# JanWosnitza/FrayTracer

Hardware: AMD Instinct MI355X
Metric: Mrays/s (primary+secondary) at 4096x4096; max per-pixel |delta| vs F# ref (delta is measured against the CPU oracle: F# parity is unpinned, DESIGN.md section 2) (higher is better)
Workload: dtype f32

## Files before the change

### fraytracer_amd/csrc/kernels.hip

```cpp
#include <hip/hip_runtime.h>

#include "../../include/fraytracer_hip.h"
#include "ft_device.h"
#include "ft_kernels.h"
#include "ft_math.h"
#include "ft_libm.h"

#define FT_CONST __attribute__((address_space(4)))
typedef const float FT_CONST* cfp;
template <class T> __device__ __forceinline__ const T FT_CONST* as_const(const T* p) {
    return (const T FT_CONST*)(p);
}

__device__ __forceinline__ f3 ld3(cfp c) { return mk3(c[0], c[1], c[2]); }
__device__ __forceinline__ FtInstr ld_instr(const FtInstr FT_CONST* q) {
    FtInstr r; r.op = q->op; r.dst = q->dst; r.src = q->src; r.type = q->type; r.count = q->count; r.data = q->data;
    r.aux = q->aux; r.flags = q->flags; r.f0 = q->f0; r.f1 = q->f1; r.pad0 = 0; r.pad1 = 0; return r;
}
typedef float v4f __attribute__((ext_vector_type(4)));
typedef uint32_t v4u __attribute__((ext_vector_type(4)));
struct ItemRegs { v4f a; v4u b; };
__device__ __forceinline__ ItemRegs ld_item(const FtItemRec FT_CONST* q) {
    ItemRegs r;
    r.a = *reinterpret_cast<const v4f FT_CONST*>(q);
// ... 214 lines not shown
        for (int j = 0; j < FT_UNROLL; ++j) {
            q[j] = ft_sphere_q(prm[j], p);
            if (CLAMP) q[j] = __builtin_fmaxf(q[j], FT_FAST_Q_MIN);
        }
#pragma unroll
        for (int j = 0; j < FT_UNROLL; ++j) sum = sum + ft_exp_fast<NEAR>(ft_strength_times_diff<PW>(si, FT_LOOP_SQRT(q[j]), prm[j].w));
    }
    for (; i < count; ++i) {
        const float4 prm = *reinterpret_cast<const float4*>(ldsC + 4 * i);
        const float q1 = ft_sphere_q(prm, p);
        sum = sum + ft_exp_fast<NEAR>(ft_strength_times_diff<PW>(si, FT_LOOP_SQRT(CLAMP ? __builtin_fmaxf(q1, FT_FAST_Q_MIN) : q1), prm.w));
    }
#ifndef FT_SQRT_5
    if (NEAR) ft_omod_off(mode, sum);
#endif
    return sum;
}

template <bool FMA, bool FQ, bool NEAR = false>
__device__ __forceinline__ float smooth_run_spheres_libm(const float* __restrict__ ldsC, uint32_t count, float si, f3 p, float sum, const ft_u64* __restrict__ tab) {
    uint32_t i = 0;
    for (; i + 4u <= count; i += 4u) {
        float4 prm[4];
        float e[4];
#pragma unroll
        for (int j = 0; j < 4; ++j) prm[j] = *reinterpret_cast<const float4*>(ldsC + 4 * (i + j));
#pragma unroll
        for (int j = 0; j < 4; ++j) {
            const float t = si * (ft_sq<FQ>(ft_sphere_q(prm[j], p)) - prm[j].w);
            e[j] = NEAR ? ft_glibc_expf_main<FMA>(t, tab) : ft_glibc_expf<FMA>(t, tab);
        }
#pragma unroll
        for (int j = 0; j < 4; ++j) sum = sum + e[j];
    }
    for (; i < count; ++i) {
        const float4 prm = *reinterpret_cast<const float4*>(ldsC + 4 * i);
        const float t = si * (ft_sq<FQ>(ft_sphere_q(prm, p)) - prm.w);
        sum = sum + (NEAR ? ft_glibc_expf_main<FMA>(t, tab) : ft_glibc_expf<FMA>(t, tab));
    }
    return sum;
}

__device__ __forceinline__ bool near_point_ok(f3 p, float nearR2) {
    const float pp = p.x * p.x + p.y * p.y + p.z * p.z;
    return __ballot(!(pp <= nearR2)) == 0ull;
}

__device__ __forceinline__ bool fast_point_ok(f3 p, bool active = true) {
    const float m = __builtin_fmaxf(__builtin_fmaxf(__builtin_fabsf(p.x), __builtin_fabsf(p.y)), __builtin_fabsf(p.z));
    const bool bad = !(m < FT_FAST_P_MAX) || p.x != p.x || p.y != p.y || p.z != p.z;
    return __ballot(active && bad) == 0ull;
}

__device__ __forceinline__ void ft_sphere_regime(const FtSceneDev& S, const f3 p, bool& fastOk, bool& nearOk) {
    fastOk = fast_point_ok(p);
    nearOk = fastOk && near_point_ok(p, S.nearR2);
}

#ifdef FT_UNION_PROFILE
__device__ unsigned long long ft_union_dbg[12];
__device__ __forceinline__ void ft_dbg_add(uint32_t k, uint32_t v) {
    __hip_atomic_fetch_add(reinterpret_cast<uint32_t*>(ft_lds) + FT_LDS_CNT_WORDS + threadIdx.x + k * FT_BLOCK, v, __ATOMIC_RELAXED, __HIP_MEMORY_SCOPE_WORKGROUP);
}
__device__ __forceinline__ bool ft_dbg_leader() { return (threadIdx.x & 63u) == (unsigned)(__ffsll((long long)__ballot(1)) - 1); }
__device__ __forceinline__ uint32_t ft_dbg_now() { unsigned long long t; asm volatile("s_memtime %0\n\ts_waitcnt lgkmcnt(0)" : "=s"(t) :: "memory"); return (uint32_t)t; }
#define FT_UDBG(k, v) ft_dbg_add(k, v)
#define FT_UDBG_WAVE(k) do { if (ft_dbg_leader()) ft_dbg_add(k, 64u); } while (0)
#define FT_UDBG_T0(v) const uint32_t v = ft_dbg_now()
#define FT_UDBG_T1(k, v) do { const uint32_t _t = ft_dbg_now(); if (ft_dbg_leader()) ft_dbg_add(k, _t - (v)); } while (0)
#else
#define FT_UDBG(k, v) do {} while (0)
#define FT_UDBG_WAVE(k) do {} while (0)
#define FT_UDBG_T0(v) do {} while (0)
#define FT_UDBG_T1(k, v) do {} while (0)
#endif

__device__ __forceinline__ uint32_t ft_grid_cell(const FtGrid FT_CONST& g, const f3 p) {
    const f3 cc = (p - mk3(g.aabbMin[0], g.aabbMin[1], g.aabbMin[2])) * mk3(g.cellSizeInv[0], g.cellSizeInv[1], g.cellSizeInv[2]);
    const int ix = ft_clamp_i(0, g.count[0] - 1, ft_floor_i(cc.x));
    const int iy = ft_clamp_i(0, g.count[1] - 1, ft_floor_i(cc.y));
    const int iz = ft_clamp_i(0, g.count[2] - 1, ft_floor_i(cc.z));
    return (uint32_t)((ix * g.count[1] + iy) * g.count[2] + iz);
}

template <bool FQ, bool CALLS, class Call>
__device__ __forceinline__ void ft_candidate(uint32_t typeData, uint32_t mat, cfp consts, const f3 p, const float* __restrict__ sd,
                                             const uint32_t* __restrict__ sl, float& d, uint32_t& l, Call call) {
    const uint32_t type = typeData & 15u, data = typeData >> 4;
    if (type == FT_PR_SLOT) { d = sd[data * FT_BLOCK]; l = sl[data * FT_BLOCK]; }
    else if (CALLS && type == FT_PR_CALL) call(data, d, l);
    else { d = prim_eval_t<FQ>(type, pool_at(consts, data), p); l = mat; }
}

template <bool FQ>
__device__ __forceinline__ void eval_union_prims(const FtSceneDev& S, const FtGrid FT_CONST& g, const f3 p,
                                           const float* __restrict__ sd, const uint32_t* __restrict__ sl,
                                           float& outD, uint32_t& outLeaf, float cap, float capBound) {
    FT_UDBG_T0(tWalk);
    const uint32_t cell = g.cellBase + ft_grid_cell(g, p);
    cfp ctr = as_const(S.cellCenters) + 3u * cell;
    const float distanceToCenter = ft_distance(mk3(ctr[0], ctr[1], ctr[2]), p);
    const uint32_t FT_CONST* cellStart = as_const(S.cellStart);
    const FtItemRec FT_CONST* items = as_const(S.items);
    cfp consts = as_const(S.consts);
    uint32_t i = cellStart[cell];
    const uint32_t end = cellStart[cell + 1];
#ifdef FT_UNION_PROFILE
    {
// ... 234 lines not shown
                if constexpr (COOP) {
                    if (fastOk && S.fastQ) eval_union_coop<true, CALLS, MATH>(S, as_const(S.grids)[in.aux], p, sd, sl, ldsC, fastOk, nearOk, d, l);
                    else eval_union_coop<false, CALLS, MATH>(S, as_const(S.grids)[in.aux], p, sd, sl, ldsC, fastOk, nearOk, d, l);
                } else
                {
                    float cap = -__builtin_inff(), capBound = 0.0f;
                    if (in.flags & FT_FLAG_LAZY) {
                        const float d1 = prim_eval(in.type, consts + in.data, p);
                        cfp bd = consts + in.count;
                        if (d1 >= epsHit) { cap = d1; capBound = ft_distance(ld3(bd), p) + bd[3]; }
                    }
                if constexpr (CALLS) {
                    if (fastOk && S.fastQ) eval_union<true, MATH>(S, as_const(S.grids)[in.aux], p, sd, sl, ldsC, fastOk, nearOk, d, l, cap, capBound);
                    else eval_union<false, MATH>(S, as_const(S.grids)[in.aux], p, sd, sl, ldsC, fastOk, nearOk, d, l, cap, capBound);
                } else {
                    if (fastOk && S.fastQ) eval_union_prims<true>(S, as_const(S.grids)[in.aux], p, sd, sl, d, l, cap, capBound);
                    else eval_union_prims<false>(S, as_const(S.grids)[in.aux], p, sd, sl, d, l, cap, capBound);
                }
                }
                *dst = d; sl[in.dst * FT_BLOCK] = l;
            }
            break;
        }
        default: break;
        }
    }
}

template <bool CALLS, int MATH, bool COOP = false>
__device__ __forceinline__ void ft_eval(const FtSceneDev& S, const f3 p, float* __restrict__ sd, uint32_t* __restrict__ sl,
                                        const float* __restrict__ ldsC, float& outD, uint32_t& outLeaf, float epsHit = __builtin_inff(),
                                        const float* __restrict__ cullRow = nullptr, uint32_t cullN = FT_CULL_NONE) {
    const bool fastOk = (S.nStage != 0 || S.fastQ != 0) && fast_point_ok(p);
    const bool nearOk = MATH == 0 && fastOk && S.nStage != 0 && near_point_ok(p, S.nearR2);
    ft_exec<true, CALLS, MATH, COOP>(S, 0u, S.nInstr, p, sd, sl, ldsC, fastOk, nearOk, epsHit, cullRow, cullN);
    outD = sd[0];
    outLeaf = sl[0];
}

#define FT_CULL_MIN 32u
__device__ __forceinline__ f3 ft_readlane3(f3 v, int l) {
    return mk3(__int_as_float(__builtin_amdgcn_readlane(__float_as_int(v.x), l)), __int_as_float(__builtin_amdgcn_readlane(__float_as_int(v.y), l)),
               __int_as_float(__builtin_amdgcn_readlane(__float_as_int(v.z), l)));
}
template <int CTRL> __device__ __forceinline__ float ft_dpp(float old, float v) {
    return __int_as_float(__builtin_amdgcn_update_dpp(__float_as_int(old), __float_as_int(v), CTRL, 0xf, 0xf, false));
}
__device__ __forceinline__ float ft_readlane_f(float v, int l) { return __int_as_float(__builtin_amdgcn_readlane(__float_as_int(v), l)); }
__device__ __forceinline__ float ft_wave_max_all(float v) {
    v = __builtin_fmaxf(v, ft_dpp<0x111>(0.0f, v)); v = __builtin_fmaxf(v, ft_dpp<0x112>(0.0f, v));
    v = __builtin_fmaxf(v, ft_dpp<0x114>(0.0f, v)); v = __builtin_fmaxf(v, ft_dpp<0x118>(0.0f, v));
    return __builtin_fmaxf(__builtin_fmaxf(ft_readlane_f(v, 15), ft_readlane_f(v, 31)), __builtin_fmaxf(ft_readlane_f(v, 47), ft_readlane_f(v, 63)));
}
__device__ __forceinline__ float ft_wave_scan_incl(float v, float& total) {
    const uint32_t lane = threadIdx.x & 63u;
    v += ft_dpp<0x111>(0.0f, v); v += ft_dpp<0x112>(0.0f, v); v += ft_dpp<0x114>(0.0f, v); v += ft_dpp<0x118>(0.0f, v);
    const float r0 = ft_readlane_f(v, 15), r1 = ft_readlane_f(v, 31), r2 = ft_readlane_f(v, 47), r3 = ft_readlane_f(v, 63);
    const float p2 = r0 + r1, p3 = p2 + r2;
    v += lane >= 48u ? p3 : (lane >= 32u ? p2 : (lane >= 16u ? r0 : 0.0f));
    total = p3 + r3;
    return v;
}
__device__ __forceinline__ float ft_wave_shift_right1(float v) { return ft_dpp<0x138>(0.0f, v); }
template <bool HELD = false>
__device__ __forceinline__ uint32_t ft_cull_children(const FtSceneDev& S, const f3 p, bool active, unsigned long long am,
                                                     const float* __restrict__ ldsC, float* __restrict__ row) {
    if (FT_WORD_AT_USE(HELD, S.cullPc) == FT_CULL_NONE) return FT_CULL_NONE;
    const FtInstr FT_CONST* in = as_const(S.instr) + S.cullPc;
    const uint32_t flags = in->flags, count = in->count;
    const float si = in->f0;
    if (in->op != FT_OP_SMOOTH_RUN || !(flags & FT_FLAG_FAST) || count < FT_CULL_MIN || !(si < 0.0f)) return FT_CULL_NONE;
    if (!fast_point_ok(p, active)) return FT_CULL_NONE;
    const uint32_t lane = threadIdx.x & 63u;
    const f3 q00 = ft_readlane3(p, __ffsll((long long)am) - 1);
    const float fx = p.x - q00.x, fy = p.y - q00.y, fz = p.z - q00.z;
    const float far2 = active ? (fx * fx + fy * fy) + fz * fz : 0.0f;
    const float farMax = ft_wave_max_all(far2);
    const unsigned long long fm = __ballot(active && far2 == farMax);
    const f3 q01 = ft_readlane3(p, __ffsll((long long)(fm != 0ull ? fm : am)) - 1);
    const f3 q0 = mk3(0.5f * (q00.x + q01.x), 0.5f * (q00.y + q01.y), 0.5f * (q00.z + q01.z));
    const float ex = p.x - q0.x, ey = p.y - q0.y, ez = p.z - q0.z;
    const float rho2 = ft_wave_max_all(active ? (ex * ex + ey * ey) + ez * ez : 0.0f);
    const float rho = __builtin_amdgcn_sqrtf(rho2) * 1.001f + 1e-6f;
    const uint32_t n = count < FT_CULL_MAX ? count : FT_CULL_MAX;
    const float4* src = reinterpret_cast<const float4*>(ldsC + in->data);
    float4* dst = reinterpret_cast<float4*>(row);
    float carry = 0.0f;
    uint32_t kept = 0;
    bool apart = true;
    for (uint32_t base = 0; base < n; base += 64u) {
        const uint32_t i = base + lane;
        const bool have = i < n;
        const float4 prm = src[have ? i : n - 1u];
        const float dx = prm.x - q0.x, dy = prm.y - q0.y, dz = prm.z - q0.z;
        const float dq = __builtin_amdgcn_sqrtf((dx * dx + dy * dy) + dz * dz);
        const float dc = dq - prm.w;
        if (__ballot(have && !(dq - rho >= 1e-5f * dq + 1e-6f)) != 0ull) apart = false;
        const float slack = 0.01f + rho;
        const float dlo = dc - slack, dhi = dc + slack;
        const float low = have ? __builtin_amdgcn_exp2f(__builtin_fmaxf(si * dhi * 1.44269504f - 0.02f, -200.0f)) : 0.0f;
        float passTotal;
        const float incl = ft_wave_scan_incl(low, passTotal);
        const float excl = ft_wave_shift_right1(incl);
        const float slow = (carry + excl) * 0.99609375f;
        const uint32_t sbits = __float_as_uint(slow);
        const float x = __builtin_fminf(__builtin_fmaxf(si * dlo * 1.44269504f, -1000.0f), 1000.0f);
        const bool drop = have && x == x && sbits >= 0x00800000u && sbits < 0x7f800000u && x + 0.02f <= (float)((int)(sbits >> 23) - 127 - 24);
        const bool keep = have && !drop;
        const unsigned long long km = __ballot(keep);
        if (keep) dst[kept + (uint32_t)__popcll(km & ((1ull << lane) - 1ull))] = prm;
        kept += (uint32_t)__popcll(km);
        carry += passTotal;
    }
    return kept | (apart ? FT_CULL_NOCLAMP : 0u);
}

template <int MATH>
__device__ __forceinline__ float ft_run_spheres(const FtSceneDev& S, const float* __restrict__ c, uint32_t count, float si, const f3 p, float sum0,
                                                bool fastOk, bool nearOk, bool noClamp = false) {
    if (MATH != 0) {
        const ft_u64* tab = ft_libm_tab(S);
        if (S.mathFma) return nearOk ? smooth_run_spheres_libm<true, true, true>(c, count, si, p, sum0, tab)
                            : fastOk ? smooth_run_spheres_libm<true, true>(c, count, si, p, sum0, tab)
                                     : smooth_run_spheres_libm<true, false>(c, count, si, p, sum0, tab);
        return nearOk ? smooth_run_spheres_libm<false, true, true>(c, count, si, p, sum0, tab)
             : fastOk ? smooth_run_spheres_libm<false, true>(c, count, si, p, sum0, tab)
                      : smooth_run_spheres_libm<false, false>(c, count, si, p, sum0, tab);
    }
    if (__builtin_expect(nearOk, 1)) {
#ifndef FT_SQRT_5
        const int pw = ft_strength_pw(si);
        if (noClamp) {
            if (pw == 2) return smooth_run_spheres_fast<true, 2, false>(c, count, si, p, sum0);
            if (pw == 1) return smooth_run_spheres_fast<true, 1, false>(c, count, si, p, sum0);
            if (pw == 3) return smooth_run_spheres_fast<true, 3, false>(c, count, si, p, sum0);
            return smooth_run_spheres_fast<true, 0, false>(c, count, si, p, sum0);
        }
        if (pw == 2) return smooth_run_spheres_fast<true, 2>(c, count, si, p, sum0);
        if (pw == 1) return smooth_run_spheres_fast<true, 1>(c, count, si, p, sum0);
        if (pw == 3) return smooth_run_spheres_fast<true, 3>(c, count, si, p, sum0);
#endif
        return smooth_run_spheres_fast<true>(c, count, si, p, sum0);
    }
    if (fastOk) return smooth_run_spheres_fast<false>(c, count, si, p, sum0);
    float acc = sum0;
    for (uint32_t i = 0; i < count; ++i) acc = acc + ft_exp(si * (ft_distance(mk3(c[4u * i], c[4u * i + 1u], c[4u * i + 2u]), p) - c[4u * i + 3u]));
    return acc;
}

template <int MATH>
__device__ __forceinline__ void ft_eval_smooth_spheres(const FtSceneDev& S, const f3 p, const float* __restrict__ ldsC,
                                                       float& outD, uint32_t& outLeaf, const float* __restrict__ cullRow = nullptr, uint32_t cullN = FT_CULL_NONE) {
    float acc = 0.0f;
    uint32_t leaf = 0;
    bool fastOk, nearOk;
    ft_sphere_regime(S, p, fastOk, nearOk);
    for (uint32_t pc = 0; pc < S.nInstr; ++pc) {
        const FtInstr FT_CONST* in = as_const(S.instr) + pc;
        const uint32_t op = in->op;
        if (op == FT_OP_SMOOTH_RUN) {
            acc = (in->flags & FT_FLAG_INIT) ? 0.0f : acc;
            const bool culled = pc == S.cullPc && cullN != FT_CULL_NONE && fastOk;
            const float* c = culled ? cullRow : ldsC + in->data;
            uint32_t n = culled ? (cullN & 0xffffu) : in->count;
            uint32_t rest = culled && in->count > FT_CULL_MAX ? in->count - FT_CULL_MAX : 0u;
            bool noClamp = culled && (cullN & FT_CULL_NOCLAMP) != 0u;
#pragma nounroll
            for (;;) {
                acc = ft_run_spheres<MATH>(S, c, n, in->f0, p, acc, fastOk, nearOk, noClamp);
                if (rest == 0u) break;
                c = ldsC + in->data + 4u * FT_CULL_MAX; n = rest; rest = 0u; noClamp = false;
            }
        }
        else if (op == FT_OP_SMOOTH_FIN) acc = -ft_log_m<MATH>(acc, S) * in->f0;
        else leaf = in->aux;
    }
    outD = acc; outLeaf = leaf;
}

#define FT_COOP_SEG 256
template <int MATH>
__device__ __forceinline__ float ft_sphere_term(const float4 prm, const f3 p, const float si, const int regime, const FtSceneDev& S) {
    const float q = ft_sphere_q(prm, p);
    if (MATH != 0) {
        const float t = si * ((regime != 0 ? ft_sq<true>(q) : sqrtf(q)) - prm.w);
        return S.mathFma ? ft_glibc_expf<true>(t, ft_libm_tab(S)) : ft_glibc_expf<false>(t, ft_libm_tab(S));
    }
    if (regime == 2) return ft_exp_fast<true>(si * (ft_sq<true>(q) - prm.w));
    if (regime == 1) return ft_exp_fast<false>(si * (ft_sq<true>(q) - prm.w));
    return ft_exp(si * (sqrtf(q) - prm.w));
}
template <int MATH>
__device__ __forceinline__ void ft_eval_smooth_spheres_packed(const FtSceneDev& S, const f3 q, const bool active, const unsigned long long am, const uint32_t nRays,
                                                              const float* __restrict__ ldsC, float* __restrict__ row, float& outD, uint32_t& outLeaf) {
    const uint32_t lane = threadIdx.x & 63u;
    const uint32_t rank = (uint32_t)__popcll(am & ((1ull << lane) - 1ull));
    const uint32_t lg = nRays <= 1u ? 6u : 6u - (32u - (uint32_t)__builtin_clz(nRays - 1u));
    const uint32_t g = 1u << lg;
    auto wave_sync = [] {
        __builtin_amdgcn_fence(__ATOMIC_RELEASE, "wavefront");
        __builtin_amdgcn_wave_barrier();
        __builtin_amdgcn_fence(__ATOMIC_ACQUIRE, "wavefront");
    };
    if (active) { row[3u * rank] = q.x; row[3u * rank + 1u] = q.y; row[3u * rank + 2u] = q.z; }
    wave_sync();
    const uint32_t G = lane >> lg, k = lane & (g - 1u);
    const bool valid = G < nRays;
    const f3 p = valid ? mk3(row[3u * G], row[3u * G + 1u], row[3u * G + 2u]) : mk3(0.0f, 0.0f, 0.0f);
    wave_sync();
// ... 268 lines not shown
    float t0, t1;
    bool ok = ft_cert_segment(S, test, o, dir, eps, len, steps, t0, t1);
    const float A = si * 1.44269504f;
    const float xt = A * (eps + S.certM);
    ok = ok && xt >= -100.0f;
    if (__ballot(ok) == 0ull) return false;
    const float thr = ft_cert_threshold(xt);
    const f3 p0 = ok ? o + dir * t0 : mk3(0.0f, 0.0f, 0.0f);
    const f3 sv = ok ? dir * (t1 - t0) : mk3(1.0f, 0.0f, 0.0f);
    const float iss = 1.0f / ft_dot(sv, sv);
    float sum = 0.0f;
    uint32_t i = 0;
    auto term = [&](const auto prm) { return __builtin_amdgcn_exp2f((__builtin_amdgcn_sqrtf(ft_seg_dist2(prm, p0, sv, iss)) - prm.w) * A); };
    if (S.certK != 0u) {
        const v4f FT_CONST* cl = reinterpret_cast<const v4f FT_CONST*>(as_const(S.certCl));
        const v4f FT_CONST* kid = cl + 2u * S.certK;
        const float mthr = thr * (0.5f / (float)S.certK);
        float all = 0.0f, rest = 0.0f;
        uint32_t mark = 0u;
        for (uint32_t k = 0; k < S.certK; ++k) {
            const float bnd = term(cl[2u * k]) * (float)__float_as_uint(cl[2u * k + 1u].x);
            all += bnd;
            if (bnd >= mthr) mark |= 1u << k;
            else rest += bnd;
        }
        const bool held = ok && all < thr, open = ok && !held;
        if (__ballot(open) == 0ull) return held;
        float exact = 0.0f;
        for (uint32_t k = 0; k < S.certK; ++k) {
            const bool mine = (mark >> k) & 1u;
            if (__ballot(open && mine) == 0ull) continue;
            const v4f r = cl[2u * k + 1u];
            const uint32_t cnt = __float_as_uint(r.x), first = __float_as_uint(r.y);
            float part = 0.0f;
            for (uint32_t j = 0; j < cnt; ++j) part += term(kid[first + j]);
            exact += mine ? part : 0.0f;
            if (__ballot(open && exact < thr) == 0ull) return held;
        }
        return held || (open && rest + exact < thr);
    }
    for (; i + 8u <= n; i += 8u) {
#pragma unroll
        for (int j = 0; j < 8; ++j) sum += term(c[i + j]);
        if (__ballot(ok && sum < thr) == 0ull) return false;
    }
    for (; i < n; ++i) sum += term(c[i]);
    return ok && sum < thr;
}

__device__ __forceinline__ int ft_axis_lane(unsigned long long mm) {
    return (mm >> 27) != 0ull ? 26 + __ffsll((long long)(mm >> 27)) : __ffsll((long long)mm) - 1;
}

__device__ __forceinline__ bool ft_bundle_certificate(const FtSceneDev& S, const float* __restrict__ ldsC, bool cand, const f3 o, const f3 dir, float eps, float len,
                                                      uint32_t steps, uint32_t minMembers) {
    float t0, t1;
    const bool mem = ft_cert_segment(S, cand, o, dir, eps, len, steps, t0, t1);
    const unsigned long long mm = __ballot(mem);
    if (mm == 0ull || (uint32_t)__popcll(mm) < minMembers) return false;
    const FtInstr FT_CONST* in = as_const(S.instr);
    const float A = in->f0 * 1.44269504f;
    const uint32_t n = in->count;
    const float4* c = reinterpret_cast<const float4*>(ldsC + in->data);
    const int ax = ft_axis_lane(mm);
    const f3 oc = ft_readlane3(o, ax), dc = ft_readlane3(dir, ax);
    const float tc0 = ft_readlane_f(t0, ax), tc1 = ft_readlane_f(t1, ax);
    const f3 g = o - oc, h = dir - dc;
    const float sl = ft_dot(g, dc) * (1.0f / ft_dot(dc, dc));
    const float ex = __builtin_fmaf(-sl, dc.x, g.x), ey = __builtin_fmaf(-sl, dc.y, g.y), ez = __builtin_fmaf(-sl, dc.z, g.z);
    const float al = __builtin_amdgcn_sqrtf(__builtin_fmaf(ez, ez, __builtin_fmaf(ey, ey, ex * ex)));
    const float bl = __builtin_amdgcn_sqrtf(__builtin_fmaf(h.z, h.z, __builtin_fmaf(h.y, h.y, h.x * h.x)));
    const float Wr = ft_wave_max_all(mem ? __builtin_fmaf(bl, t1, al) : 0.0f);
    const float epsMax = ft_wave_max_all(mem ? eps : 0.0f);
    const float Rc = (S.escR + epsMax + S.certClip) * 1.001f;
    const float W = Wr * 1.001f + (1e-6f + 4e-6f * Rc);
    const float xt = A * (epsMax + S.certM);
    if (!(W <= S.escR) || !(xt >= -100.0f)) return false;
    const float dLo = ft_wave_max_all(mem ? __builtin_fmaxf(tc1 - (sl + t0), 0.0f) : 0.0f);
    const float dHi = ft_wave_max_all(mem ? __builtin_fmaxf((sl + t1) - tc0, 0.0f) : 0.0f);
    const float i0 = (tc1 - dLo) - 4e-6f * Rc, i1 = (tc0 + dHi) + 4e-6f * Rc;
    const f3 p0 = oc + dc * i0, sv = dc * (i1 - i0);
    const float iss = 1.0f / ft_dot(sv, sv);
    const float thr = ft_cert_threshold(xt);
    const uint32_t lane = threadIdx.x & 63u;
    float sum = 0.0f;
    for (uint32_t base = 0; base < n; base += 64u) {
        const uint32_t i = base + lane;
        const float4 prm = c[i < n ? i : n - 1u];
        const float term = __builtin_amdgcn_exp2f((__builtin_amdgcn_sqrtf(ft_seg_dist2(prm, p0, sv, iss)) - (prm.w + W)) * A);
        sum += i < n ? term : 0.0f;
    }
    float total;
    ft_wave_scan_incl(sum, total);
    return mem && total < thr;
}

__device__ __forceinline__ bool ft_occlusion_certificate(const FtRenderArgs& a, const float* __restrict__ ldsC, bool cand, const f3 o, const f3 dir, float eps, float len,
                                                         uint32_t steps) {
    const FtSceneDev& S = a.S;
    const f3 w = o - mk3(S.escC[0], S.escC[1], S.escC[2]);
    const float dd = ft_dot(dir, dir);
    const bool ok = cand && a.occ.b >= 0.0f && S.escR >= 0.0f && eps >= a.occ.epsMin && eps <= S.escR && len > 0.0f && len < 1e9f && dd >= 0.81f && dd <= 1.000001f &&
                    ft_dot(w, w) <= S.certRho2 && steps < FT_STEP_CAP / 2u;
    const unsigned long long mm = __ballot(ok);
    if (mm == 0ull) return false;
    const FtInstr FT_CONST* in = as_const(S.instr);
    const uint32_t n = in->count;
    const float si = in->f0;
    const float4* c = reinterpret_cast<const float4*>(ldsC + in->data);
    const float tEnd = len * a.occ.lenInv;
    const int ax = ft_axis_lane(mm);
    const f3 oc = ft_readlane3(o, ax), dc = ft_readlane3(dir, ax);
    const float tc = ft_readlane_f(tEnd, ax), idc = 1.0f / ft_dot(dc, dc);
    const uint32_t lane = threadIdx.x & 63u;
    auto approach = [](const f3 p, const f3 q, const f3 e, const float ie, const float tMaxi, float& t) {
        const float vx = p.x - q.x, vy = p.y - q.y, vz = p.z - q.z;
        t = __builtin_amdgcn_fmed3f(__builtin_fmaf(vz, e.z, __builtin_fmaf(vy, e.y, vx * e.x)) * ie, 0.0f, tMaxi);
        const float ex = __builtin_fmaf(-t, e.x, vx), ey = __builtin_fmaf(-t, e.y, vy), ez = __builtin_fmaf(-t, e.z, vz);
        return __builtin_amdgcn_sqrtf(__builtin_fmaf(ez, ez, __builtin_fmaf(ey, ey, ex * ex)));
    };
    float best = 0.0f, tAx;
    uint32_t bi = 0u;
    for (uint32_t base = 0; base < n; base += 64u) {
        const uint32_t i = base + lane;
        const float4 prm = c[i < n ? i : n - 1u];
        const float nr = (prm.w + a.occ.near) - approach(mk3(prm.x, prm.y, prm.z), oc, dc, idc, tc, tAx);
        if (i < n && nr > best) { best = nr; bi = i; }
    }
    const float nearest = ft_wave_max_all(best);
    if (!(nearest > 0.0f)) return false;
    const int src = __ffsll((long long)__ballot(best == nearest)) - 1;
    const float4 sp = c[(uint32_t)__builtin_amdgcn_readlane((int)bi, src)];
    (void)approach(mk3(sp.x, sp.y, sp.z), oc, dc, idc, tc, tAx);
    const f3 y = oc + dc * tAx;
    const float A = si * 1.44269504f;
    float sum = 0.0f;
    for (uint32_t base = 0; base < n; base += 64u) {
        const uint32_t i = base + lane;
        const float4 prm = c[i < n ? i : n - 1u];
        const float dx = prm.x - y.x, dy = prm.y - y.y, dz = prm.z - y.z;
        const float term = __builtin_amdgcn_exp2f((__builtin_amdgcn_sqrtf(__builtin_fmaf(dz, dz, __builtin_fmaf(dy, dy, dx * dx))) - prm.w) * A);
        sum += i < n ? term : 0.0f;
    }
    float total;
    ft_wave_scan_incl(sum, total);
    const float D = __builtin_amdgcn_logf(total) * (-0.693147181f / si);
    const float ie = 1.0f / eps, idd = 1.0f / dd;
    float t;
    bool holds = false;
    {
        const float dist = approach(mk3(sp.x, sp.y, sp.z), o, dir, idd, tEnd, t);
        const float nSteps = __builtin_fmaf(t, ie, 2.0f), hitM = __builtin_fmaf(a.occ.e, nSteps, a.occ.b);
        holds = t <= a.occ.reach && nSteps < 131072.0f && hitM <= a.occ.cap && (dist + hitM) * 1.001f < sp.w;
    }
    {
        const float dist = approach(y, o, dir, idd, tEnd, t);
        const float nSteps = __builtin_fmaf(t, ie, 2.0f), hitM = __builtin_fmaf(a.occ.e, nSteps, a.occ.b);
        holds = holds || (t <= a.occ.reach && nSteps < 131072.0f && hitM <= a.occ.cap && (dist + hitM) * 1.001f < D);
    }
    return ok && holds;
}

__device__ __forceinline__ int first_step_from_cache(LaneState& s) {
    if (s.len <= 0.0f) return 0;
    const float d = *ft_sh(FT_SH_D0);
    if (d != d) { ft_flag(1u); return 2; }
    if (d < s.eps) return 1;
    s.o = s.o + s.dir * d;
    s.len = s.len - d;
    s.steps = 1;
    return 0;
}

struct FtLit { f3 lint, ldir; };
__device__ __forceinline__ FtLit ft_light_at(const uint32_t type, const f3 lv, const f3 lc, const f3 hp) {
    f3 lint = lc, ldir = lv;
    if (type != FT_LIGHT_DIRECTIONAL) { ldir = ft_normalize(lv - hp); lint = lint / ft_length2(lv - hp); }
    return FtLit{lint, ldir};
}

template <bool EXT, int FORM = FT_FORM_FRAME, bool LEAN = false>
__device__ __forceinline__ void settle(const FtRenderArgs& a, LaneState& s) {
// ... 284 lines not shown
            const unsigned long long idle = __ballot(s.phase == PH_IDLE);
            if (idle == 0ull) break;
            if ((uint32_t)__popcll(idle) < a.refillMin && __ballot(s.phase >= PH_MARCH) != 0ull) break;
            if (chunkNext == chunkEnd) {
                if (exhausted) break;
                const FtRenderArgs& u = FT_ARGS_AT_USE(LEAN, a);
                if (ORDER && u.tileCost != nullptr && lane == 0) {
                    const uint32_t t = tileSt[0];
                    if (t < (u.nJobs >> 6)) u.tileCost[t] = waveEvals - tileSt[TILE_EVALS];
                    tileSt[0] = 0xffffffffu;
                }
                uint32_t base = 0, take = u.chunk;
                if (lane == 0) {
                    if (u.shrink1 < u.nJobs) {
                        const uint32_t cur = __hip_atomic_load(u.counter, __ATOMIC_RELAXED, __HIP_MEMORY_SCOPE_AGENT);
                        take = cur >= u.shrink2 ? u.chunk / 4u : (cur >= u.shrink1 ? u.chunk / 2u : u.chunk);
                    }
                    base = atomicAdd(u.counter, take);
                }
                base = __builtin_amdgcn_readfirstlane(base);
                const uint32_t took = (uint32_t)__builtin_amdgcn_readfirstlane((int)take);
                if (base >= u.nJobs) { exhausted = true; break; }
                chunkNext = base;
                chunkEnd = (u.nJobs - base < took) ? u.nJobs : base + took;
                if (ORDER && u.tileCost != nullptr) {
                    uint32_t tile = base >> 6;
                    if (u.tileOrder != nullptr) {
                        tile = (uint32_t)__builtin_amdgcn_readfirstlane((int)u.tileOrder[tile]);
                        chunkNext = tile << 6; chunkEnd = chunkNext + 64u;
                    }
                    if (lane == 0) { tileSt[0] = tile; tileSt[TILE_EVALS] = waveEvals; }
                }
            }
            uint32_t avail = chunkEnd - chunkNext;
            if (VIEWS && a.mode == 0u) {
                const uint32_t jobsPerView = a.jobsPerPlane * (EXT ? a.spp : 1u);
                const uint32_t v = chunkNext / jobsPerView, viewEnd = (v + 1u) * jobsPerView;
                if (viewEnd - chunkNext < avail) avail = viewEnd - chunkNext;
                cfp c = as_const(a.views) + 12u * v;
                vc.o = ld3(c); vc.fw = ld3(c + 3); vc.up = ld3(c + 6); vc.rt = ld3(c + 9);
                vc.d = ft_readlane_f(dCam, (int)v); vc.leaf = (uint32_t)__builtin_amdgcn_readlane((int)leafCam, (int)v);
            }
            const uint32_t nIdle = (uint32_t)__popcll(idle);
            const uint32_t rank = (uint32_t)__popcll(idle & ((1ull << lane) - 1ull));
            if (s.phase == PH_IDLE && rank < avail) { s.job = chunkNext + rank; start_job<EXT, FORM, LEAN>(a, s, camKnown, dCam, leafCam, vc); }
            chunkNext += (nIdle < avail) ? nIdle : avail;
        }
        if (s.phase == PH_IDLE && exhausted && chunkNext == chunkEnd) s.phase = PH_DONE;
        if (__ballot(s.phase != PH_DONE) == 0ull) break;

        if (VARIANT == 1 && FT_WORD_AT_USE(LEAN, a.occPeriod) != 0u && waveEvals % a.occPeriod == 0u) {
            const bool cand = s.phase == PH_SHADOW && s.steps - a.occFrom < a.occPeriod && (!EXT || !s.inside());
            if ((uint32_t)__popcll(__ballot(cand)) >= a.occMin) {
                const bool hit = ft_occlusion_certificate(FT_ARGS_AT_USE(LEAN, a), ldsC + 0, cand, s.o, s.dir, s.eps, s.len, s.steps);
                if (hit) { ft_count(FT_C_HITS); s.lidx += 1; s.phase = PH_LIGHTS; settle<EXT, FORM, LEAN>(a, s); }
                if (__ballot(hit) != 0ull && __ballot(s.phase >= PH_MARCH) == 0ull) continue;
            }
        }

        if (VARIANT == 1 && FT_WORD_AT_USE(LEAN, a.cert) != 0u) {
            bool ends = false;
            if (FT_WORD_AT_USE(LEAN, a.bundlePeriod) != 0u && waveEvals % a.bundlePeriod == 0u) {
#pragma unroll 1
                for (uint32_t ph = SHADE ? PH_SHADOW : PH_MARCH; ph <= PH_SHADOW; ph += PH_SHADOW - PH_MARCH) {
                    const bool cand = s.phase == ph && (ph == PH_MARCH || s.steps >= a.bundleShadow) && (!EXT || !s.inside());
                    if ((uint32_t)__popcll(__ballot(cand)) < a.bundleMin) continue;
                    if (ft_bundle_certificate(FT_ARGS_AT_USE(LEAN, a).S, ldsC + 0, cand, s.o, s.dir, s.eps, s.len, s.steps, a.bundleMin)) ends = true;
                }
            }
            const bool due = !ends && (s.phase == PH_MARCH || s.phase == PH_SHADOW) && s.steps >= s.certAt && (!EXT || !s.inside());
            bool tried = false;
            if ((uint32_t)__popcll(__ballot(due)) >= a.certMin) {
                tried = true;
                const FtRenderArgs& u = FT_ARGS_AT_USE(LEAN, a);
                const bool holds = ft_miss_certificate(u.S, ldsC + 0, due, s.o, s.dir, s.eps, s.len, s.steps);
                if (due) {
                    if (holds) ends = true;
                    else s.certAt = u.certRepeat != 0u ? s.steps + u.certRepeat : 0xffffffffu;
                }
            }
            if (ends) { s.len = -1.0f; settle<EXT, FORM, LEAN>(a, s); }
            if ((tried || __ballot(ends) != 0ull) && __ballot(s.phase >= PH_MARCH) == 0ull) continue;
        }

        const bool active = s.phase >= PH_MARCH;
        waveEvals += 1;
        FT_UDBG_T0(tRound);
        auto query_point = [&]() {
            f3 q = s.o;
            if (!SHADE && s.phase >= PH_NX && s.phase <= PH_NC) {
                const f3 base = s.o + s.dir * (-s.eps);
                const float h = s.eps * 0.125f;
                q = base;
                if (s.phase == PH_NX) q.x = base.x + h;
                if (s.phase == PH_NY) q.y = base.y + h;
                if (s.phase == PH_NZ) q.z = base.z + h;
            }
            return q;
        };
        const unsigned long long am = __ballot(active);
        const bool camRound = __ballot(s.phase == PH_CAM) != 0ull;
        if (LEAN) { if (!camRound) ft_wave_word_add(waveSt + ST_EVALS, (uint32_t)__popcll(am)); }
        else if (!camRound) nEvals += (uint32_t)__popcll(am);
        const bool coop = (uint32_t)__popcll(am) <= a.tailK;
        float dCoop = 0.0f; uint32_t leafCoop = 0;
        if (coop && am != 0ull) {
            const f3 qm = query_point();
            if (VARIANT == 1) {
                ft_eval_smooth_spheres_packed<MATH>(a.S, qm, active, am, (uint32_t)__popcll(am), ldsC, coopRow, dCoop, leafCoop);
                if (LEAN) { if (!camRound) ft_wave_word_add(waveSt + ST_COOP, (uint32_t)__popcll(am)); }
                else if (!camRound) coopEvals += (uint32_t)__popcll(am);
            } else {
                unsigned long long m = am;
                while (m != 0ull) {
                    const int L = __ffsll((long long)m) - 1;
                    m &= m - 1ull;
                    const f3 qL = ft_readlane3(qm, L);
                    float dL; uint32_t leafL;
                    if (VARIANT == 3) ft_eval_carved<K, true>(a.S, a.carve, qL, dL, leafL, __builtin_inff());
                    else ft_eval<VARIANT == 2, MATH, true>(a.S, qL, sd, sl, ldsC, dL, leafL);
                    if ((int)lane == L) { dCoop = dL; leafCoop = leafL; }
                    if (!camRound) coopEvals += 1;
                }
            }
        }
        uint32_t cullN = FT_CULL_NONE;
        if (VARIANT != 3 && FT_WORD_AT_USE(LEAN, a.cull) != 0u && !coop && am != 0ull) {
            cullN = ft_cull_children<LEAN>(a.S, query_point(), active, am, ldsC, coopRow);
            if (cullN != FT_CULL_NONE) {
                const uint32_t cnt = (as_const(a.S.instr) + a.S.cullPc)->count;
                const uint32_t looked = cnt < FT_CULL_MAX ? cnt : FT_CULL_MAX;
                const uint32_t total = looked * (uint32_t)__popcll(am) >> 6, skipped = (looked - (cullN & 0xffffu)) * (uint32_t)__popcll(am) >> 6;
                if (LEAN) { ft_wave_word_add(waveSt + ST_CULL_TOTAL, total); ft_wave_word_add(waveSt + ST_CULL_SKIPPED, skipped); }
                else { cullTotal += total; cullSkipped += skipped; }
            }
        }
        if (active) {
            float d; uint32_t leaf;
            FT_UDBG_T0(tEval);
            if (coop) { d = dCoop; leaf = leafCoop; }
            else {
                const f3 q = query_point();
                if (VARIANT == 1) ft_eval_smooth_spheres<MATH>(a.S, q, ldsC, d, leaf, coopRow, cullN);
                else if (VARIANT == 3) ft_eval_carved<K>(a.S, a.carve, q, d, leaf, a.lazy == 0u ? __builtin_inff() : s.eps);
                else ft_eval<VARIANT == 2, MATH>(a.S, q, sd, sl, ldsC, d, leaf,
                                                  (EXT && s.inside()) || a.lazy == 0u ? __builtin_inff() : s.eps, coopRow, cullN);
            }
            FT_UDBG_T1(5, tEval); FT_UDBG_WAVE(6);
            if (EXT) d = __uint_as_float(__float_as_uint(d) ^ (s.xs & 0x80000000u));

            const uint32_t ph = SHADE ? (uint32_t)PH_SHADOW : s.phase;
            switch (ph) {
            case PH_MARCH:
            case PH_SHADOW:
            case PH_AO: {
                bool miss = false;
                if (d != d) { ft_flag(1u); miss = true; }
                else if (d < s.eps) {
                    if (ph == PH_MARCH) {
                        ft_count(FT_C_HITP); s.leaf = leaf; s.phase = PH_NX;
                        if (EXT && a.mode == 2u) {
                            float* o = a.out + 10ull * s.outIdx;
                            write_ray(o, s.o, s.dir, s.len, s.eps);
                            o[8] = d; reinterpret_cast<int32_t*>(o)[9] = 1;
                            s.phase = PH_IDLE;
                        }
                    }
                    else if (ph == PH_SHADOW) { ft_count(FT_C_HITS); s.lidx += 1; s.phase = PH_LIGHTS; }
                    else { s.xs += 1u; s.phase = PH_AONEXT; }
                } else {
                    s.o = s.o + s.dir * d;
                    s.len = s.len - d;
                    s.steps += 1;
                    if (s.steps >= FT_STEP_CAP) { ft_flag(4u); miss = true; }
                }
                if (miss) s.len = -1.0f;
                break;
            }
            case PH_CAM:
                if (VIEWS) { dCam = d; leafCam = leaf; }
                else { dCam = ft_readlane_f(d, 0); leafCam = (uint32_t)__builtin_amdgcn_readlane((int)leaf, 0); }
                camKnown = true;
                s.phase = PH_IDLE;
                break;
            case PH_NX: *ft_sh(FT_SH_NRM) = d; s.phase = PH_NY; break;
            case PH_NY: *ft_sh(FT_SH_NRM + 1) = d; s.phase = PH_NZ; break;
            case PH_NZ: *ft_sh(FT_SH_NRM + 2) = d; s.phase = PH_NC; break;
            case PH_NC: {
                *ft_sh(FT_SH_D0) = d;
                const f3 nrm = ft_normalize(sh_get3(FT_SH_NRM) - splat3(d));
                const f3 hp = s.o + s.dir * (-s.eps);
                sh_set3(FT_SH_NRM, nrm);
                sh_set3(FT_SH_HP, hp);
                sh_set3(FT_SH_LACC, ft_background(a));
                s.lidx = 0;
                s.phase = PH_LIGHTS;
// ... 759 lines not shown
```

Before: 1208.

## Add lean wave reductions, early-exit bundle certificate, and lean cull pass

Adds a LEAN variant of wave-wide max using DPP row_bcast in inline asm, plus a lean inclusive scan that applies row offsets with masked DPP moves instead of per-lane selects. In the LEAN cull path, the loop is split into full 64-wide chunks and a tail, and the 'apart' tracking becomes a ballot accumulator. The fast-point check in the sphere evaluator is skipped when culling already validated it. The bundle certificate returns early once any lane's sum crosses the threshold. These target cross-lane reduction overhead and redundant checks in the hot march loop. The inline asm with s_nop hazard padding carries correctness risk.

```diff
diff --git a/fraytracer_amd/csrc/kernels.hip b/fraytracer_amd/csrc/kernels.hip
--- a/fraytracer_amd/csrc/kernels.hip
+++ b/fraytracer_amd/csrc/kernels.hip
@@ -290,8 +290,9 @@
     return __ballot(active && bad) == 0ull;
 }
 
-__device__ __forceinline__ void ft_sphere_regime(const FtSceneDev& S, const f3 p, bool& fastOk, bool& nearOk) {
-    fastOk = fast_point_ok(p);
+template <bool LEAN = false>
+__device__ __forceinline__ void ft_sphere_regime(const FtSceneDev& S, const f3 p, bool& fastOk, bool& nearOk, bool known = false) {
+    fastOk = (LEAN && known) || fast_point_ok(p);
     nearOk = fastOk && near_point_ok(p, S.nearR2);
 }
 
@@ -632,12 +633,38 @@
     v = __builtin_fmaxf(v, ft_dpp<0x114>(0.0f, v)); v = __builtin_fmaxf(v, ft_dpp<0x118>(0.0f, v));
     return __builtin_fmaxf(__builtin_fmaxf(ft_readlane_f(v, 15), ft_readlane_f(v, 31)), __builtin_fmaxf(ft_readlane_f(v, 47), ft_readlane_f(v, 63)));
 }
+__device__ __forceinline__ float ft_wave_max_all_lean(float v) {
+    uint32_t r;
+    asm("s_nop 1\n\tv_max_f32_dpp %1, %1, %1 row_shr:1 row_mask:0xf bank_mask:0xf bound_ctrl:1\n\t"
+        "s_nop 1\n\tv_max_f32_dpp %1, %1, %1 row_shr:2 row_mask:0xf bank_mask:0xf bound_ctrl:1\n\t"
+        "s_nop 1\n\tv_max_f32_dpp %1, %1, %1 row_shr:4 row_mask:0xf bank_mask:0xf bound_ctrl:1\n\t"
+        "s_nop 1\n\tv_max_f32_dpp %1, %1, %1 row_shr:8 row_mask:0xf bank_mask:0xf bound_ctrl:1\n\t"
+        "s_nop 1\n\tv_max_f32_dpp %1, %1, %1 row_bcast:15 row_mask:0xa bank_mask:0xf\n\t"
+        "s_nop 1\n\tv_max_f32_dpp %1, %1, %1 row_bcast:31 row_mask:0xc bank_mask:0xf\n\t"
+        "s_nop 1\n\tv_readlane_b32 %0, %1, 63\n\t"
+        "s_nop 1"
+        : "=s"(r), "+v"(v));
+    return __uint_as_float(r);
+}
+template <bool LEAN> __device__ __forceinline__ float ft_wave_max(float v) { return LEAN ? ft_wave_max_all_lean(v) : ft_wave_max_all(v); }
 __device__ __forceinline__ float ft_wave_scan_incl(float v, float& total) {
     const uint32_t lane = threadIdx.x & 63u;
     v += ft_dpp<0x111>(0.0f, v); v += ft_dpp<0x112>(0.0f, v); v += ft_dpp<0x114>(0.0f, v); v += ft_dpp<0x118>(0.0f, v);
     const float r0 = ft_readlane_f(v, 15), r1 = ft_readlane_f(v, 31), r2 = ft_readlane_f(v, 47), r3 = ft_readlane_f(v, 63);
     const float p2 = r0 + r1, p3 = p2 + r2;
     v += lane >= 48u ? p3 : (lane >= 32u ? p2 : (lane >= 16u ? r0 : 0.0f));
+    total = p3 + r3;
+    return v;
+}
+__device__ __forceinline__ float ft_wave_scan_incl_lean(float v, float& total) {
+    v += ft_dpp<0x111>(0.0f, v); v += ft_dpp<0x112>(0.0f, v); v += ft_dpp<0x114>(0.0f, v); v += ft_dpp<0x118>(0.0f, v);
+    const float r0 = ft_readlane_f(v, 15), r1 = ft_readlane_f(v, 31), r2 = ft_readlane_f(v, 47), r3 = ft_readlane_f(v, 63);
+    const float p2 = r0 + r1, p3 = p2 + r2;
+    int off = 0;
+    off = __builtin_amdgcn_update_dpp(off, __float_as_int(r0), 0xe4, 0x2, 0xf, false);
+    off = __builtin_amdgcn_update_dpp(off, __float_as_int(p2), 0xe4, 0x4, 0xf, false);
+    off = __builtin_amdgcn_update_dpp(off, __float_as_int(p3), 0xe4, 0x8, 0xf, false);
+    v += __int_as_float(off);
     total = p3 + r3;
     return v;
 }
@@ -655,18 +682,48 @@
     const f3 q00 = ft_readlane3(p, __ffsll((long long)am) - 1);
     const float fx = p.x - q00.x, fy = p.y - q00.y, fz = p.z - q00.z;
     const float far2 = active ? (fx * fx + fy * fy) + fz * fz : 0.0f;
-    const float farMax = ft_wave_max_all(far2);
+    const float farMax = ft_wave_max<HELD>(far2);
     const unsigned long long fm = __ballot(active && far2 == farMax);
     const f3 q01 = ft_readlane3(p, __ffsll((long long)(fm != 0ull ? fm : am)) - 1);
     const f3 q0 = mk3(0.5f * (q00.x + q01.x), 0.5f * (q00.y + q01.y), 0.5f * (q00.z + q01.z));
     const float ex = p.x - q0.x, ey = p.y - q0.y, ez = p.z - q0.z;
-    const float rho2 = ft_wave_max_all(active ? (ex * ex + ey * ey) + ez * ez : 0.0f);
+    const float rho2 = ft_wave_max<HELD>(active ? (ex * ex + ey * ey) + ez * ez : 0.0f);
     const float rho = __builtin_amdgcn_sqrtf(rho2) * 1.001f + 1e-6f;
     const uint32_t n = count < FT_CULL_MAX ? count : FT_CULL_MAX;
     const float4* src = reinterpret_cast<const float4*>(ldsC + in->data);
     float4* dst = reinterpret_cast<float4*>(row);
     float carry = 0.0f;
     uint32_t kept = 0;
+    if (HELD) {
+        const float slack = 0.01f + rho;
+        unsigned long long close = 0ull;
+        auto pass = [&](const float4 prm, const bool have) __attribute__((always_inline)) {
+            const float dx = prm.x - q0.x, dy = prm.y - q0.y, dz = prm.z - q0.z;
+            const float dq = __builtin_amdgcn_sqrtf((dx * dx + dy * dy) + dz * dz);
+            const float dc = dq - prm.w;
+            close |= __builtin_amdgcn_ballot_w64(have && !(dq - rho >= 1e-5f * dq + 1e-6f));
+            const float dlo = dc - slack, dhi = dc + slack;
+            const float low = have ? __builtin_amdgcn_exp2f(__builtin_fmaxf(si * dhi * 1.44269504f - 0.02f, -200.0f)) : 0.0f;
+            float passTotal;
+            const float incl = ft_wave_scan_incl_lean(low, passTotal);
+            const float excl = __int_as_float(__builtin_amdgcn_mov_dpp(__float_as_int(incl), 0x138, 0xf, 0xf, true));
+            const float slow = (carry + excl) * 0.99609375f;
+            const uint32_t sbits = __float_as_uint(slow);
+            const float x = __builtin_fminf(__builtin_fmaxf(si * dlo * 1.44269504f, -1000.0f), 1000.0f);
+            const bool drop = have && x == x && sbits >= 0x00800000u && sbits < 0x7f800000u && x + 0.02f <= (float)((int)(sbits >> 23) - 127 - 24);
+            const bool keep = have && !drop;
+            const unsigned long long km = __ballot(keep);
+            if (keep) dst[kept + __builtin_amdgcn_mbcnt_hi((uint32_t)(km >> 32), __builtin_amdgcn_mbcnt_lo((uint32_t)km, 0u))] = prm;
+            kept += (uint32_t)__popcll(km);
+            carry += passTotal;
+        };
+        const float4* mine = src + lane;
+        const uint32_t whole = n & ~63u;
+        uint32_t base = 0;
+        for (; base < whole; base += 64u) pass(mine[base], true);
+        if (base < n) { const bool have = base + lane < n; pass(src[have ? base + lane : n - 1u], have); }
+        return kept | (close == 0ull ? FT_CULL_NOCLAMP : 0u);
+    }
     bool apart = true;
     for (uint32_t base = 0; base < n; base += 64u) {
         const uint32_t i = base + lane;
@@ -728,13 +785,13 @@
     return acc;
 }
 
-template <int MATH>
+template <int MATH, bool LEAN = false>
 __device__ __forceinline__ void ft_eval_smooth_spheres(const FtSceneDev& S, const f3 p, const float* __restrict__ ldsC,
                                                        float& outD, uint32_t& outLeaf, const float* __restrict__ cullRow = nullptr, uint32_t cullN = FT_CULL_NONE) {
     float acc = 0.0f;
     uint32_t leaf = 0;
     bool fastOk, nearOk;
-    ft_sphere_regime(S, p, fastOk, nearOk);
+    ft_sphere_regime<LEAN>(S, p, fastOk, nearOk, cullN != FT_CULL_NONE);
     for (uint32_t pc = 0; pc < S.nInstr; ++pc) {
         const FtInstr FT_CONST* in = as_const(S.instr) + pc;
         const uint32_t op = in->op;
@@ -1109,6 +1166,7 @@
     return (mm >> 27) != 0ull ? 26 + __ffsll((long long)(mm >> 27)) : __ffsll((long long)mm) - 1;
 }
 
+template <bool LEAN = false>
 __device__ __forceinline__ bool ft_bundle_certificate(const FtSceneDev& S, const float* __restrict__ ldsC, bool cand, const f3 o, const f3 dir, float eps, float len,
                                                       uint32_t steps, uint32_t minMembers) {
     float t0, t1;
@@ -1127,14 +1185,14 @@
     const float ex = __builtin_fmaf(-sl, dc.x, g.x), ey = __builtin_fmaf(-sl, dc.y, g.y), ez = __builtin_fmaf(-sl, dc.z, g.z);
     const float al = __builtin_amdgcn_sqrtf(__builtin_fmaf(ez, ez, __builtin_fmaf(ey, ey, ex * ex)));
     const float bl = __builtin_amdgcn_sqrtf(__builtin_fmaf(h.z, h.z, __builtin_fmaf(h.y, h.y, h.x * h.x)));
-    const float Wr = ft_wave_max_all(mem ? __builtin_fmaf(bl, t1, al) : 0.0f);
-    const float epsMax = ft_wave_max_all(mem ? eps : 0.0f);
+    const float Wr = ft_wave_max<LEAN>(mem ? __builtin_fmaf(bl, t1, al) : 0.0f);
+    const float epsMax = ft_wave_max<LEAN>(mem ? eps : 0.0f);
     const float Rc = (S.escR + epsMax + S.certClip) * 1.001f;
     const float W = Wr * 1.001f + (1e-6f + 4e-6f * Rc);
     const float xt = A * (epsMax + S.certM);
     if (!(W <= S.escR) || !(xt >= -100.0f)) return false;
-    const float dLo = ft_wave_max_all(mem ? __builtin_fmaxf(tc1 - (sl + t0), 0.0f) : 0.0f);
-    const float dHi = ft_wave_max_all(mem ? __builtin_fmaxf((sl + t1) - tc0, 0.0f) : 0.0f);
+    const float dLo = ft_wave_max<LEAN>(mem ? __builtin_fmaxf(tc1 - (sl + t0), 0.0f) : 0.0f);
+    const float dHi = ft_wave_max<LEAN>(mem ? __builtin_fmaxf((sl + t1) - tc0, 0.0f) : 0.0f);
     const float i0 = (tc1 - dLo) - 4e-6f * Rc, i1 = (tc0 + dHi) + 4e-6f * Rc;
     const f3 p0 = oc + dc * i0, sv = dc * (i1 - i0);
     const float iss = 1.0f / ft_dot(sv, sv);
@@ -1146,12 +1204,14 @@
         const float4 prm = c[i < n ? i : n - 1u];
         const float term = __builtin_amdgcn_exp2f((__builtin_amdgcn_sqrtf(ft_seg_dist2(prm, p0, sv, iss)) - (prm.w + W)) * A);
         sum += i < n ? term : 0.0f;
+        if (LEAN && __ballot(sum >= thr) != 0ull) return false;
     }
     float total;
     ft_wave_scan_incl(sum, total);
     return mem && total < thr;
 }
 
+template <bool LEAN = false>
 __device__ __forceinline__ bool ft_occlusion_certificate(const FtRenderArgs& a, const float* __restrict__ ldsC, bool cand, const f3 o, const f3 dir, float eps, float len,
                                                          uint32_t steps) {
     const FtSceneDev& S = a.S;
@@ -1184,7 +1244,7 @@
         const float nr = (prm.w + a.occ.near) - approach(mk3(prm.x, prm.y, prm.z), oc, dc, idc, tc, tAx);
         if (i < n && nr > best) { best = nr; bi = i; }
     }
-    const float nearest = ft_wave_max_all(best);
+    const float nearest = ft_wave_max<LEAN>(best);
     if (!(nearest > 0.0f)) return false;
     const int src = __ffsll((long long)__ballot(best == nearest)) - 1;
     const float4 sp = c[(uint32_t)__builtin_amdgcn_readlane((int)bi, src)];
@@ -1575,7 +1635,7 @@
         if (VARIANT == 1 && FT_WORD_AT_USE(LEAN, a.occPeriod) != 0u && waveEvals % a.occPeriod == 0u) {
             const bool cand = s.phase == PH_SHADOW && s.steps - a.occFrom < a.occPeriod && (!EXT || !s.inside());
             if ((uint32_t)__popcll(__ballot(cand)) >= a.occMin) {
-                const bool hit = ft_occlusion_certificate(FT_ARGS_AT_USE(LEAN, a), ldsC + 0, cand, s.o, s.dir, s.eps, s.len, s.steps);
+                const bool hit = ft_occlusion_certificate<LEAN>(FT_ARGS_AT_USE(LEAN, a), ldsC + 0, cand, s.o, s.dir, s.eps, s.len, s.steps);
                 if (hit) { ft_count(FT_C_HITS); s.lidx += 1; s.phase = PH_LIGHTS; settle<EXT, FORM, LEAN>(a, s); }
                 if (__ballot(hit) != 0ull && __ballot(s.phase >= PH_MARCH) == 0ull) continue;
             }
@@ -1588,7 +1648,7 @@
                 for (uint32_t ph = SHADE ? PH_SHADOW : PH_MARCH; ph <= PH_SHADOW; ph += PH_SHADOW - PH_MARCH) {
                     const bool cand = s.phase == ph && (ph == PH_MARCH || s.steps >= a.bundleShadow) && (!EXT || !s.inside());
                     if ((uint32_t)__popcll(__ballot(cand)) < a.bundleMin) continue;
-                    if (ft_bundle_certificate(FT_ARGS_AT_USE(LEAN, a).S, ldsC + 0, cand, s.o, s.dir, s.eps, s.len, s.steps, a.bundleMin)) ends = true;
+                    if (ft_bundle_certificate<LEAN>(FT_ARGS_AT_USE(LEAN, a).S, ldsC + 0, cand, s.o, s.dir, s.eps, s.len, s.steps, a.bundleMin)) ends = true;
                 }
             }
             const bool due = !ends && (s.phase == PH_MARCH || s.phase == PH_SHADOW) && s.steps >= s.certAt && (!EXT || !s.inside());
@@ -1664,7 +1724,7 @@
             if (coop) { d = dCoop; leaf = leafCoop; }
             else {
                 const f3 q = query_point();
-                if (VARIANT == 1) ft_eval_smooth_spheres<MATH>(a.S, q, ldsC, d, leaf, coopRow, cullN);
+                if (VARIANT == 1) ft_eval_smooth_spheres<MATH, LEAN>(a.S, q, ldsC, d, leaf, coopRow, cullN);
                 else if (VARIANT == 3) ft_eval_carved<K>(a.S, a.carve, q, d, leaf, a.lazy == 0u ? __builtin_inff() : s.eps);
                 else ft_eval<VARIANT == 2, MATH>(a.S, q, sd, sl, ldsC, d, leaf,
                                                   (EXT && s.inside()) || a.lazy == 0u ? __builtin_inff() : s.eps, coopRow, cullN);
```

Result: faster. 1234, median of 6 (+2.2%).
